# kkoutini/PaSST

Hardware: AMD Instinct MI355X
Metric: clips/s (10s@32k) fwd+bwd passt_s (higher is better)
Workload: dtype bf16; 1 GPU; passt_s_swa_p16_128_ap476 train step (mel front end + mixup + fwd + BCE + bwd + adamw), 768/12/12, 474 tokens (s_patchout_t=40,f=4), random-init weights; global_batch=64, per_gpu_batch=64, parallelism=dp1, gemm_launch=persistent, 256 workgroups, input=waveform (B,1,320000) f32 resident in HBM

## Files before the change

### include/passt_amd.h

```cpp
#ifndef PASST_AMD_H
#define PASST_AMD_H

#include <stdint.h>

#ifdef __cplusplus
extern "C" {
#endif

#define PA_ABI_VERSION 6

enum { PA_F32 = 0, PA_BF16 = 1 };

enum {
    PA_OK = 0,
    PA_EINVAL = -1,
    PA_EUNSUPPORTED = -2,
    PA_ELAUNCH = -3,
    PA_ECOMM = -4
};

int pa_abi_version(void);
const char* pa_error_string(int code);
const char* pa_last_hip_error(void);

// ... 83 lines not shown
    PA_EPI_RESID = 2,
    PA_EPI_DGELU = 3,
    PA_EPI_PARTIAL = 4
};
typedef struct {
    int32_t dtype;
    int32_t epilogue;
    int32_t M, N, K;
    int32_t lda, ldb;
    const void* A;
    const void* B;
    const float* bias;
    const float* resid;
    int32_t ldr;
    int32_t row_mod, out_batch_rows, out_row_off;
    const void* aux;
    int32_t ldaux;
    float* out_f32;
    int32_t ldo32;
    void* out_lp;
    int32_t ldolp;
    void* out_lp2;
    int32_t ldolp2;
    int32_t split_k;
    int32_t tune;
    float* colsum_out;
    float* colsum_ws;
    int32_t colsum_accumulate;
    int32_t reserved;
    int32_t colscale_n;
    float colscale;
} pa_gemm_args;
#define PA_GEMM_BLOCKED_PRE 0x100
#define PA_GEMM_NO_PERSIST 0x400
#define PA_GEMM_EPILOGUE_V3 0x1000
#define PA_GEMM_COLSUM_DEFER 0x2000
int pa_gemm_blocked_pre_ok(int M, int N, int K);
int64_t pa_gemm_blocked_pre_elems(int M, int N);
int64_t pa_gemm_colsum_ws_floats(int M, int N);
int pa_gemm_nt(const pa_gemm_args* a, void* stream);
int pa_gemm_nt_splitk_plan(int M, int N, int K, int epilogue, int dtype);
int64_t pa_gemm_nt_splitk_ws_floats(int M, int N, int K, int epilogue, int dtype);
int pa_gemm_nt_splitk(const pa_gemm_args* a, float* ws, int64_t ws_floats, void* stream);
int pa_gemm_nt_rowscale(const pa_gemm_args* a, const float* rowscale, void* stream);
int pa_gemm_nt_splitk_rowscale(const pa_gemm_args* a, const float* rowscale, float* ws, int64_t ws_floats, void* stream);
int pa_gemm_tn(const pa_gemm_args* a, void* stream);
#define PA_TN_BATCH_MAX 4
#ifndef PA_TN_STEP_ROWS
#define PA_TN_STEP_ROWS 48
#endif
int pa_gemm_tn_step_rows(void);
int pa_gemm_tn_batched(const pa_gemm_args* a, int n, void* stream);
int pa_gemm_tn_batched_plan(const pa_gemm_args* a, int n, int n_long, int long_steps, void* stream);
int pa_gather_rows(const void* in, const int32_t* idx, int n_idx, int64_t row_bytes, void* out, void* stream);
int pa_scatter_rows(const void* in, const int32_t* idx, int n_idx, int64_t row_bytes, void* out, void* stream);
int pa_tail_inject(const float* rows, const int32_t* idx, int n_idx, const float* add0, const float* add1, float* dx,
                   void* dx_lp, int dtype, int M, int D, void* stream);
int pa_zero2d(void* ptr, int64_t pitch_bytes, int64_t width_bytes, int64_t rows, void* stream);
int pa_reduce_partials(const float* partial, int splits, int64_t n, float* out, int accumulate,
                       void* stream);
#define PA_REDUCE_BATCH_MAX 12
#define PA_REDUCE_SLABS 0
#define PA_REDUCE_ROWS 1
typedef struct pa_reduce_desc {
    const float* partial;
    float* out;
    int64_t n;
    int32_t splits;
    int32_t accumulate;
    int64_t pitch;
    int32_t mode;
    int32_t reserved;
} pa_reduce_desc;
int pa_reduce_partials_batched(const pa_reduce_desc* d, int n, void* stream);
int pa_gemm_last_colsum_rows(void);
int pa_rowsum(const void* in, int dtype, int R, int C, int ld, float* out, int accumulate,
              void* stream);
int64_t pa_colsum_ws_floats(int R, int C);
int pa_colsum(const void* in, int dtype, int R, int C, int ld, float* out, int accumulate, float* ws,
              void* stream);
int pa_colsum_f32(const float* in, int R, int C, int ld, float* out, int accumulate, void* stream);

#define PA_ATTN_Q_PRESCALED 1
#define PA_ATTN_BWD_TWO_PASS 2
#define PA_ATTN_BWD_SINGLE_PASS 4
#define PA_ATTN_BWD_SINGLE_PASS_W16 8
int pa_attention_fwd(const void* qkv, int ldqkv, void* o, int ldo, float* lse, int B, int H, int N, int nq,
                     float scale, int dtype, int flags, void* stream);
int pa_attention_fwd_varlen(const void* qkv, int ldqkv, void* o, int ldo, float* lse, const int32_t* cu_tok, int B, int H,
                            int max_N, int nq, float scale, int dtype, int flags, void* stream);
int pa_attention_probs(const void* qkv, int ldqkv, const float* lse, float* out, const int32_t* cu_tok, const int64_t* out_off,
                       int B, int H, int N , int nq, int head_mean, float scale, int dtype, int flags,
                       void* stream);
#define PA_ATTN_PGRAD_GRAD 0
#define PA_ATTN_PGRAD_CAM 1
int pa_attention_probs_grad(const void* qkv, int ldqkv, const float* lse, const void* d_o, int ldo, int do_compact, float* out,
                            const int32_t* cu_tok, const int64_t* out_off, int B, int H, int N , int nq,
                            int head_mean, int mode, float scale, int dtype, int flags, void* stream);
#define PA_ATTN_ROLLOUT_ATTN 0
#define PA_ATTN_ROLLOUT_CAM 1
#define PA_ATTN_ROLLOUT_MAX_ROWS 4
int64_t pa_attention_rollout_ws_floats(int64_t total_tok, int B, int N , int nq, int nr, int slices);
int pa_attention_rollout(const void* qkv, int ldqkv, const float* lse, const void* d_o, int ldo, int do_compact, const float* r_in,
                         float* r_out, float* ws, const int32_t* cu_tok, int64_t total_tok, int B, int H,
                         int N , int nq, int nr, int mode, int slices, float a, float b_, float g_scale,
                         float scale, int dtype, int flags, void* stream);
// ... 118 lines not shown
```

### passt_amd/_lib.py

```python
import ctypes as C
import os

_HERE = os.path.dirname(os.path.abspath(__file__))
LIB_PATH = os.path.join(_HERE, "libpasst_amd.so")
LIB_PATH = os.environ.get("PASST_AMD_LIB", LIB_PATH)

PA_F32, PA_BF16 = 0, 1
EPI_STORE, EPI_GELU, EPI_RESID, EPI_DGELU, EPI_PARTIAL = 0, 1, 2, 3, 4

vp, i32, i64, f32 = C.c_void_p, C.c_int32, C.c_int64, C.c_float


class MelParams(C.Structure):
    _fields_ = [("n_fft", i32), ("hop", i32), ("n_mels", i32), ("n_frames", i32),
                ("preemph", f32), ("mel_low", f32), ("inv_mel_delta", f32), ("log_eps", f32),
                ("out_add", f32), ("out_scale", f32),
                ("fmask_start", i32), ("fmask_end", i32), ("tmask_start", i32), ("tmask_end", i32)]


class MelClipParams(C.Structure):
    _fields_ = [("mel_low", f32), ("inv_mel_delta", f32),
                ("fmask_start", i32), ("fmask_end", i32), ("tmask_start", i32), ("tmask_end", i32)]


# ... 9 lines not shown

class ReduceDesc(C.Structure):
    _fields_ = [("partial", vp), ("out", vp), ("n", i64), ("splits", i32), ("accumulate", i32), ("pitch", i64), ("mode", i32),
                ("reserved", i32)]


class StageDesc(C.Structure):
    _fields_ = [("src", vp), ("dst", vp), ("dst_t", vp), ("rows", i32), ("cols", i32), ("tile_begin", i32), ("reserved", i32)]


class AdamwStageDesc(C.Structure):
    _fields_ = [("offset", i64), ("dst", vp), ("dst_t", vp), ("rows", i32), ("cols", i32), ("tile_begin", i32), ("reserved", i32)]


SIGNATURES = {
    "pa_abi_version": (i32, []),
    "pa_error_string": (C.c_char_p, [i32]),
    "pa_last_hip_error": (C.c_char_p, []),
    "pa_mel_num_frames": (i32, [i32, i32]),
    "pa_mel_frontend_fwd": (i32, [vp, i32, i32, vp, vp, vp, vp, C.POINTER(MelParams), vp]),
    "pa_mel_frontend_fwd_varlen": (i32, [vp, i32, i32, vp, vp, vp, vp, vp, i32, f32, C.POINTER(MelParams), vp]),
    "pa_mel_frontend_bwd": (i32, [vp, i32, i32, vp, vp, vp, vp, vp, vp, i64, C.POINTER(MelParams), vp]),
    "pa_mel_frontend_bwd_varlen": (i32, [vp, i32, i32, vp, vp, vp, vp, vp, i32, vp, vp, i64, C.POINTER(MelParams), vp]),
    "pa_mel_frontend_fwd_varlen_aug": (i32, [vp, i32, i32, vp, vp, vp, vp, vp, i32, f32, C.POINTER(MelParams), vp, vp]),
    "pa_mel_frontend_bwd_varlen_aug": (i32, [vp, i32, i32, vp, vp, vp, vp, vp, i32, vp, vp, i64, C.POINTER(MelParams), vp, vp]),
    "pa_convert_f32": (i32, [vp, vp, i64, i32, vp]),
    "pa_convert_f32_rowscale": (i32, [vp, vp, vp, i32, i32, i32, vp]),
    "pa_convert_to_f32": (i32, [vp, i32, vp, i64, vp]),
    "pa_transpose": (i32, [vp, i32, i32, i32, i32, vp, i32, i32, vp]),
    "pa_stage_weights": (i32, [vp, i32, i32, i32, vp]),
    "pa_layernorm_fwd": (i32, [vp, vp, vp, vp, i32, vp, vp, i32, i32, f32, vp]),
    "pa_layernorm_bwd_ws_floats": (i64, [i32, i32]),
    "pa_layernorm_bwd": (i32, [vp, i32, vp, vp, vp, vp, vp, vp, vp, vp, vp, vp, i32, vp, i32, i32, vp]),
    "pa_layernorm_bwd_rows": (i32, [i32]),
    "pa_layernorm_bwd_partial": (i32, [vp, i32, vp, vp, vp, vp, vp, vp, vp, vp, i32, i32, vp]),
    "pa_layernorm_bwd2": (i32, [vp, i32, vp, vp, vp, vp, vp, vp, vp, vp, vp, vp, vp, i32, vp, i32, i32, vp]),
    "pa_layernorm_bwd2_partial": (i32, [vp, i32, vp, vp, vp, vp, vp, vp, vp, vp, vp, i32, i32, vp]),
    "pa_layernorm_bwd_rowscale": (i32, [vp, i32, vp, vp, vp, vp, vp, vp, vp, vp, vp, vp, vp, vp, i32, vp, i32, i32, vp]),
    "pa_layernorm_bwd_partial_rowscale": (i32, [vp, i32, vp, vp, vp, vp, vp, vp, vp, vp, vp, vp, i32, i32, vp]),
    "pa_tail_inject": (i32, [vp, vp, i32, vp, vp, vp, vp, i32, i32, i32, vp]),
    "pa_gemm_last_colsum_rows": (i32, []),
    "pa_gemm_colsum_ws_floats": (i64, [i32, i32]),
    "pa_gemm_blocked_pre_ok": (i32, [i32, i32, i32]),
    "pa_gemm_blocked_pre_elems": (i64, [i32, i32]),
    "pa_gemm_nt": (i32, [C.POINTER(GemmArgs), vp]),
    "pa_gemm_nt_splitk_plan": (i32, [i32, i32, i32, i32, i32]),
    "pa_gemm_nt_splitk_ws_floats": (i64, [i32, i32, i32, i32, i32]),
    "pa_gemm_nt_splitk": (i32, [C.POINTER(GemmArgs), vp, i64, vp]),
    "pa_gemm_nt_rowscale": (i32, [C.POINTER(GemmArgs), vp, vp]),
    "pa_gemm_nt_splitk_rowscale": (i32, [C.POINTER(GemmArgs), vp, vp, i64, vp]),
    "pa_gemm_tn": (i32, [C.POINTER(GemmArgs), vp]),
    "pa_gemm_tn_batched": (i32, [C.POINTER(GemmArgs), i32, vp]),
    "pa_gemm_tn_batched_plan": (i32, [C.POINTER(GemmArgs), i32, i32, i32, vp]),
    "pa_gemm_tn_step_rows": (i32, []),
    "pa_reduce_partials_batched": (i32, [C.POINTER(ReduceDesc), i32, vp]),
    "pa_colsum_ws_floats": (i64, [i32, i32]),
    "pa_colsum": (i32, [vp, i32, i32, i32, i32, vp, i32, vp, vp]),
    "pa_reduce_partials": (i32, [vp, i32, i64, vp, i32, vp]),
    "pa_rowsum": (i32, [vp, i32, i32, i32, i32, vp, i32, vp]),
    "pa_colsum_f32": (i32, [vp, i32, i32, i32, vp, i32, vp]),
    "pa_attention_fwd": (i32, [vp, i32, vp, i32, vp, i32, i32, i32, i32, f32, i32, i32, vp]),
    "pa_attention_fwd_varlen": (i32, [vp, i32, vp, i32, vp, vp, i32, i32, i32, i32, f32, i32, i32, vp]),
    "pa_attention_probs": (i32, [vp, i32, vp, vp, vp, vp, i32, i32, i32, i32, i32, f32, i32, i32, vp]),
    "pa_attention_probs_grad": (i32, [vp, i32, vp, vp, i32, i32, vp, vp, vp, i32, i32, i32, i32, i32, i32, f32, i32, i32, vp]),
    "pa_attention_rollout_ws_floats": (i64, [i64, i32, i32, i32, i32, i32]),
    "pa_attention_rollout": (i32, [vp, i32, vp, vp, i32, i32, vp, vp, vp, vp, i64, i32, i32, i32, i32, i32, i32, i32, f32, f32, f32, f32,
                                   i32, i32, vp]),
    "pa_attention_bwd_ws_floats": (i64, [i32, i32, i32]),
    "pa_attention_bwd": (i32, [vp, i32, vp, vp, i32, vp, vp, vp, i32, i32, i32, i32, i32, f32, i32, i32, vp]),
    "pa_attention_bwd_varlen_ws_floats": (i64, [i64, i32, i32, i32]),
    "pa_attention_bwd_varlen": (i32, [vp, i32, vp, vp, i32, vp, vp, vp, i32, vp, i32, i32, i32, i32, f32, i32, i32, vp]),
    "pa_gather_rows": (i32, [vp, vp, i32, i64, vp, vp]),
    "pa_scatter_rows": (i32, [vp, vp, i32, i64, vp, vp]),
    "pa_zero2d": (i32, [vp, i64, i64, i64, vp]),
    "pa_patch_gather": (i32, [vp, i32, i32, i32, vp, vp, i32, i32, i32, i32, vp, i32, vp]),
    "pa_patch_pos_table": (i32, [vp, vp, i32, vp, i32, vp, vp, i32, i32, i32, vp, vp, vp, vp, vp, i32, i32, vp]),
    "pa_patch_gather_varlen": (i32, [vp, i32, i32, i32, vp, vp, vp, i32, i32, i32, i32, vp, i32, vp]),
    "pa_patch_pos_table_varlen": (i32, [vp, vp, i32, vp, i32, vp, vp, i32, i32, vp, vp, vp, vp, vp]),
    "pa_patch_input_bwd_varlen": (i32, [vp, i32, vp, i32, i32, i32, i32, i32, i32, vp, vp]),
    "pa_patch_bwd_varlen": (i32, [vp, i32, i32, vp, i32, i32, i32, vp, vp, vp, vp, vp, vp, i32, vp]),
    "pa_patch_input_bwd_rows": (i32, [vp, i32, i32, vp, i32, i32, i32, i32, i32, i32, i32, vp, vp]),
    "pa_patch_bwd_rows": (i32, [vp, i32, i32, vp, vp, vp, i32, i32, i32, i32, vp, vp, vp, vp, vp, vp, i32, vp]),
    "pa_patch_bwd": (i32, [vp, i32, i32, i32, vp, vp, i32, i32, i32, i32, vp, vp, vp, vp, vp, vp, vp, i32, vp, i32, vp]),
    "pa_patch_input_bwd_ws_ints": (i64, [i32, i32, i32, i32, i32]),
    "pa_patch_input_bwd": (i32, [vp, i32, i32, i32, vp, vp, i32, i32, i32, i32, i32, vp, vp, vp]),
    "pa_head_pre_fwd": (i32, [vp, i32, i32, i32, vp, vp, f32, vp, vp, f32, vp, vp, vp, vp]),
    "pa_linear_f32_fwd": (i32, [vp, vp, vp, vp, i32, i32, i32, vp]),
    "pa_linear_f32_bwd": (i32, [vp, vp, vp, vp, vp, vp, i32, i32, i32, i32, vp]),
    "pa_head_pre_bwd": (i32, [vp, vp, vp, vp, i32, i32, i32, vp, vp, vp, vp, vp, vp]),
    "pa_bce_fwd_bwd": (i32, [vp, vp, i32, i32, f32, vp, vp, vp, vp]),
    "pa_ce_mixup_fwd_bwd": (i32, [vp, vp, vp, vp, i32, i32, f32, vp, vp, vp, vp]),
    "pa_mixup": (i32, [vp, vp, vp, vp, i32, i64, vp]),
    "pa_adamw": (i32, [vp, vp, vp, vp, i64, f32, f32, f32, f32, f32, i32, vp]),
    "pa_adamw_dev": (i32, [vp, vp, vp, vp, i64, vp, vp]),
    "pa_adamw_stage": (i32, [vp, vp, vp, vp, vp, i32, i32, i32, f32, f32, f32, f32, f32, i32, vp, vp]),
    "pa_adamw_stage_groups": (i32, [vp, vp, vp, vp, vp, vp, i32, i32, i32, f32, f32, f32, f32, f32, i32, vp, vp]),
    "pa_adamw_groups": (i32, [vp, vp, vp, vp, vp, vp, i32, i32, f32, f32, f32, f32, f32, i32, vp, vp]),
    "pa_grad_norm_partials": (i64, [i64]),
    "pa_grad_accum_sumsq": (i32, [vp, vp, i32, i64, vp, vp]),
    "pa_clip_coef": (i32, [vp, i32, f32, vp, vp]),
    "pa_adamw_clip": (i32, [vp, vp, vp, vp, i64, f32, f32, f32, f32, f32, i32, vp, vp, vp]),
    "pa_adamw_stage_clip": (i32, [vp, vp, vp, vp, vp, vp, i32, i32, i32, f32, f32, f32, f32, f32, i32, vp, vp, vp]),
    "pa_adamw_hyper": (None, [f32, f32, f32, f32, f32, i32, C.POINTER(f32)]),
    "pa_sgd": (i32, [vp, vp, i64, f32, vp]),
    "pa_swa_update": (i32, [vp, vp, i64, i32, vp]),
    "pa_wave_augment": (i32, [vp, i32, i64, vp, vp, vp, vp, vp, vp, vp, i64, vp]),
    "pa_ir_conv_plan": (i32, [i32, C.POINTER(i32), C.POINTER(i32)]),
    "pa_ir_bank_floats": (i64, [i32, i32]),
    "pa_ir_bank_prepare": (i32, [vp, i32, i32, vp, vp, vp]),
    "pa_wave_ir_convolve": (i32, [vp, i32, i64, vp, vp, vp, vp, i32, i32, vp, i64, i64, vp, vp]),
    "pa_eval_append": (i32, [vp, vp, vp, i32, i32, i64, i64, i32, vp, vp, vp]),
    "pa_eval_ws_bytes": (i64, [i32, i64]),
    "pa_eval_rank": (i32, [vp, vp, i32, i64, i64, vp, vp, vp, vp, vp, vp, vp]),
    "pa_comm_unique_id": (i32, [vp]),
    "pa_comm_init": (i32, [vp, i32, i32, C.POINTER(vp)]),
    "pa_allreduce_bucket": (i32, [vp, vp, i64, i32, vp]),
    "pa_comm_destroy": (i32, [vp]),
    "pa_comm_info": (i32, [vp, C.POINTER(i32), C.POINTER(i32), C.POINTER(i32), C.POINTER(i32)]),
    "pa_comm_last_error": (C.c_char_p, []),
}
GEMM_BLOCKED_PRE = 0x100
GEMM_NO_PERSIST = 0x400
GEMM_COLSUM_DEFER = 0x2000
REDUCE_SLABS, REDUCE_ROWS = 0, 1
GEMM_EPILOGUE_V3 = 0x1000
COMM_ID_BYTES = 128
EVAL_SIGMOID, EVAL_RAW = 0, 1
EVAL_EXCLUDED, EVAL_NEG, EVAL_POS, EVAL_NAN = 0, 1, 2, 3

_lib = None


class PasstAmdError(RuntimeError):
    pass


def load():
    global _lib
    if _lib is not None:
        return _lib
    if not os.path.isfile(LIB_PATH):
        raise PasstAmdError(
            f"{LIB_PATH} not found: the HIP extension is not built.  Run "
            "`make -C passt_amd/csrc` (needs hipcc, --offload-arch=gfx950).  passt_amd has no CPU fallback.")
    lib = C.CDLL(LIB_PATH)
    for name, (res, args) in SIGNATURES.items():
        fn = getattr(lib, name)
        fn.restype, fn.argtypes = res, args
    if lib.pa_abi_version() != 6:
        raise PasstAmdError("libpasst_amd.so ABI version mismatch; rebuild")
    _lib = lib
    return lib


def compile_opaque(fn):
    import functools

    import torch
    try:
        ef = torch._C._dynamo.eval_frame
        set_eval_frame = ef.set_eval_frame
        skip = ef._FrameExecStrategy(ef._FrameAction.SKIP, ef._FrameAction.DEFAULT)
    except AttributeError:
        return torch.compiler.disable(fn)

    @functools.wraps(fn)
    def opaque_forward(*args, **kwargs):
        prior = set_eval_frame(None)
        try:
            return fn(*args, **kwargs)
        finally:
            set_eval_frame(prior)

    ef.set_code_exec_strategy(opaque_forward.__code__, skip)
    opaque_forward._torchdynamo_disable = True
# ... 15 lines not shown
```

### passt_amd/csrc/gemm.hip

```cpp
#include <algorithm>
#include <cstring>
#include <type_traits>

#include "pa_mma.h"

namespace pa {

static constexpr int NT_GROUP_M = 4;
static constexpr int BM = 128, BN = 128, KB = 128;
static constexpr int TILE_BYTES = BM * KB;
static constexpr int GEMM_LDS = 2 * 2 * TILE_BYTES;

#ifdef PA_PROBE
__device__ unsigned long long* g_probe_buf = nullptr;
static constexpr int PROBE_SLOTS = 512;
#define PA_PROBE_STAMP(cond, idx)                                                                             \
    do {                                                                                                      \
        if ((cond) && (wave & 3) == 0 && lane == 0 && (idx) < PROBE_SLOTS)                                    \
            ((unsigned long long*)(smem + G::LDS))[(wave >> 2) * PROBE_SLOTS + (idx)] = __builtin_amdgcn_s_memtime(); \
    } while (0)
#define PA_PROBE_FLAG(a, bit) (((a).reserved >> (bit)) & 1)
#define PA_PROBE_STAMP_TN(cond, idx)                                                                          \
    do {                                                                                                      \
        if ((cond) && (wave & 3) == 0 && lane == 0 && (idx) < PROBE_SLOTS)                                    \
            ((unsigned long long*)(smem + TN_LDS))[(wave >> 2) * PROBE_SLOTS + (idx)] = __builtin_amdgcn_s_memtime(); \
    } while (0)
#else
#define PA_PROBE_STAMP(cond, idx) do {} while (0)
#define PA_PROBE_STAMP_TN(cond, idx) do {} while (0)
#define PA_PROBE_FLAG(a, bit) 0
#endif


static constexpr int SLAB_BYTES = 32 * 68 * 4;

static int finish_gemm_colsum(const pa_gemm_args& a, int rows, hipStream_t st);

template <int EPI, int TM> __host__ __device__ constexpr int aux_depth() {
    return EPI == PA_EPI_DGELU ? TM : (EPI == PA_EPI_RESID ? (TM <= 3 ? TM : 2) : 0);
}

template <int EPI>
__device__ __forceinline__ void load_bias8(const pa_gemm_args& a, int n0, int wc, int lane, float (&bias8)[8]) {
    const int ncol = n0 + wc * 64 + (lane & 7) * 8;
#pragma unroll
    for (int e = 0; e < 8; ++e) bias8[e] = 0.f;
    if constexpr (EPI != PA_EPI_PARTIAL && EPI != PA_EPI_DGELU) {
        if (a.bias && ncol < a.N) {
            const f32x4 lo = *(const f32x4*)(a.bias + ncol), hi = *(const f32x4*)(a.bias + ncol + 4);
#pragma unroll
            for (int e = 0; e < 4; ++e) { bias8[e] = lo[e]; bias8[4 + e] = hi[e]; }
        }
    }
}

// ... 1645 lines not shown
    gemm_tn_stagger_item(a, tiles_n, xcd_swizzle(blockIdx.x, nwg), blockIdx.y, steps_per_split);
}

struct TnBatch {
    pa_gemm_args a[PA_TN_BATCH_MAX];
    int32_t first[PA_TN_BATCH_MAX + 1];
    int32_t tiles_n[PA_TN_BATCH_MAX], nwg[PA_TN_BATCH_MAX], per[PA_TN_BATCH_MAX];
    int32_t tfirst[PA_TN_BATCH_MAX + 1];
    int32_t n, order;
};
__global__ __launch_bounds__(512) void gemm_tn_stagger_batched_kernel(const TnBatch b) {
    int p = 0, t, split;
    if (b.order == 1) {
        const int logical = xcd_swizzle(blockIdx.x, b.first[b.n]);
        const int tiles_all = b.tfirst[b.n];
        split = logical / tiles_all;
        t = logical - split * tiles_all;
        while (p + 1 < b.n && t >= b.tfirst[p + 1]) ++p;
        t -= b.tfirst[p];
    } else {
        while (p + 1 < b.n && (int)blockIdx.x >= b.first[p + 1]) ++p;
        const int item = blockIdx.x - b.first[p];
        split = item / b.nwg[p];
        t = xcd_swizzle(item - split * b.nwg[p], b.nwg[p]);
    }
    gemm_tn_stagger_item(b.a[p], b.tiles_n[p], t, split, b.per[p]);
}

struct TnPlan {
    pa_gemm_args a[PA_TN_BATCH_MAX];
    int32_t tiles_n[PA_TN_BATCH_MAX];
    int32_t tfirst[PA_TN_BATCH_MAX + 1];
    int32_t n, n_long, long_steps, steps;
};
__global__ __launch_bounds__(512) void gemm_tn_stagger_plan_kernel(const TnPlan b) {
    const int tiles_all = b.tfirst[b.n], nlong = tiles_all * b.n_long;
    int g, t;
    if ((int)blockIdx.x < nlong) {
        const int logical = xcd_swizzle(blockIdx.x, nlong);
        g = logical / tiles_all;
        t = logical - g * tiles_all;
    } else {
        g = b.n_long;
        t = xcd_swizzle(blockIdx.x - nlong, tiles_all);
    }
    int p = 0;
    while (p + 1 < b.n && t >= b.tfirst[p + 1]) ++p;
    t -= b.tfirst[p];
    const pa_gemm_args& a = b.a[p];
    const int st_begin = g * b.long_steps;
    const int nsteps = g < b.n_long ? b.long_steps : b.steps - st_begin;
    gemm_tn_stagger_range(a, b.tiles_n[p], t, st_begin, nsteps, a.out_f32 + (int64_t)g * a.M * a.ldo32, a.ldo32,
                          a.colsum_ws ? a.colsum_ws + (int64_t)g * a.M : nullptr);
}

static int launch_gemm_tn_stagger(const pa_gemm_args& a, hipStream_t st) {
#ifdef PA_PROBE
    constexpr int LDS = TN_LDS + 2 * PROBE_SLOTS * 8;
#else
    constexpr int LDS = TN_LDS;
#endif
    const int tiles_m = (int)cdiv(a.M, 256), tiles_n = (int)cdiv(a.N, 256);
    const int nwg = tiles_m * tiles_n;
    const int steps = (int)cdiv(a.K, TN_ROWS);
    const int per = (int)cdiv(steps, a.split_k);
    static signed char lds_attr[64] = {0};
    (void)lds_attr_on_this_device((const void*)gemm_tn_stagger_kernel, LDS, lds_attr);
    hipLaunchKernelGGL(gemm_tn_stagger_kernel, dim3(nwg, a.split_k), dim3(512), LDS, st, a, tiles_n, nwg, per);
    return check_launch();
}

template <typename T>
static int launch_gemm_tn(const pa_gemm_args& a, hipStream_t st) {
    const int tiles_m = (int)cdiv(a.M, BM), tiles_n = (int)cdiv(a.N, BN);
    const int nwg = tiles_m * tiles_n;
    const int steps = (int)cdiv(a.K, TNGeom<T>::MROWS);
    const int per = (int)cdiv(steps, a.split_k);
    static signed char lds_attr[64] = {0};
    (void)lds_attr_on_this_device((const void*)gemm_tn_kernel<T>, GEMM_LDS, lds_attr);
    hipLaunchKernelGGL((gemm_tn_kernel<T>), dim3(nwg, a.split_k), dim3(256), GEMM_LDS, st, a, tiles_n, nwg, per);
    return check_launch();
}

template <typename T>
__global__ __launch_bounds__(256) void colsum_stage1_kernel(const T* __restrict__ in, int R, int C, int ld,
                                                            float* __restrict__ part, int rows_per_block) {
    __shared__ float red[32][65];
    const int tx = threadIdx.x & 7, ty = threadIdx.x >> 3;
    const int c0 = blockIdx.x * 64 + tx * 8;
    const int r_begin = blockIdx.y * rows_per_block, r_end = min(R, r_begin + rows_per_block);
    float s[8];
#pragma unroll
    for (int e = 0; e < 8; ++e) s[e] = 0.f;
    for (int r = r_begin + ty; r < r_end; r += 32) {
        float v[8];
        if (c0 < C) {
            load8<T>(in + (int64_t)r * ld + c0, v);
#pragma unroll
            for (int e = 0; e < 8; ++e) s[e] += v[e];
        }
    }
#pragma unroll
    for (int e = 0; e < 8; ++e) red[ty][tx * 8 + e] = s[e];
    __syncthreads();
    if (threadIdx.x < 64) {
        float t = 0.f;
// ... 489 lines not shown
        tiles += pb->nwg[p];
        same_split = same_split && x.split_k == a[0].split_k;
    }
    pb->first[n] = total;
    pb->tfirst[n] = tiles;
    pb->n = n;
    pb->order = (a[0].tune != 2 && same_split) ? 1 : 0;
#ifdef PA_PROBE
    constexpr int LDS = TN_LDS + 2 * PROBE_SLOTS * 8;
#else
    constexpr int LDS = TN_LDS;
#endif
    static signed char lds_attr[64] = {0};
    (void)lds_attr_on_this_device((const void*)gemm_tn_stagger_batched_kernel, LDS, lds_attr);
    hipLaunchKernelGGL(gemm_tn_stagger_batched_kernel, dim3(total), dim3(512), LDS, (hipStream_t)stream, batch);
    return check_launch();
}

extern "C" int pa_gemm_tn_batched_plan(const pa_gemm_args* a, int n, int n_long, int long_steps, void* stream) {
    if (!a || n < 1 || n > PA_TN_BATCH_MAX || n_long < 1 || long_steps < 1) return PA_EINVAL;
    TnPlan plan;
    TnPlan* pb = &plan;
    int64_t tiles = 0;
    for (int p = 0; p < n; ++p) {
        const pa_gemm_args& x = a[p];
        if (!x.A || !x.B || !x.out_f32 || x.M <= 0 || x.N <= 0 || x.K <= 0 || x.split_k != n_long + 1) return PA_EINVAL;
        if (x.dtype != PA_BF16 || x.epilogue != PA_EPI_PARTIAL) return PA_EUNSUPPORTED;
        if ((x.lda * 2) % 16 || (x.ldb * 2) % 16 || x.ldo32 % 4 || x.M < 8 || x.N < 8 || x.N % 8 || x.M % 8) return PA_EUNSUPPORTED;
        if (x.K != a[0].K) return PA_EUNSUPPORTED;
        pb->a[p] = x;
        pb->tiles_n[p] = (int)cdiv(x.N, 256);
        pb->tfirst[p] = (int)tiles;
        tiles += cdiv(x.M, 256) * pb->tiles_n[p];
    }
    const int steps = (int)cdiv(a[0].K, TN_ROWS);
    if ((int64_t)n_long * long_steps >= steps) return PA_EINVAL;
    if (tiles * (n_long + 1) > INT32_MAX) return PA_EUNSUPPORTED;
    pb->tfirst[n] = (int)tiles;
    pb->n = n;
    pb->n_long = n_long;
    pb->long_steps = long_steps;
    pb->steps = steps;
#ifdef PA_PROBE
    constexpr int LDS = TN_LDS + 2 * PROBE_SLOTS * 8;
#else
    constexpr int LDS = TN_LDS;
#endif
    static signed char lds_attr[64] = {0};
    (void)lds_attr_on_this_device((const void*)gemm_tn_stagger_plan_kernel, LDS, lds_attr);
    hipLaunchKernelGGL(gemm_tn_stagger_plan_kernel, dim3((unsigned)(tiles * (n_long + 1))), dim3(512), LDS, (hipStream_t)stream, plan);
    return check_launch();
}

namespace pa {
struct ReduceBatch {
    pa_reduce_desc d[PA_REDUCE_BATCH_MAX];
    int32_t n;
};
__global__ __launch_bounds__(256) void reduce_partials_batched_kernel(const ReduceBatch b) {
    const pa_reduce_desc& d = b.d[blockIdx.y];
    if (d.mode == PA_REDUCE_ROWS) {
        __shared__ float red[16][17];
        const int cx = threadIdx.x & 15, ry = threadIdx.x >> 4;
        for (int64_t c0 = (int64_t)blockIdx.x * 16; c0 < d.n; c0 += (int64_t)gridDim.x * 16) {
            const int64_t k = c0 + cx;
            float s = 0.f, s1 = 0.f, s2 = 0.f, s3 = 0.f;
            if (k < d.n) {
                int r = ry;
                for (; r + 48 < d.splits; r += 64) {
                    s += d.partial[(int64_t)r * d.pitch + k];
                    s1 += d.partial[(int64_t)(r + 16) * d.pitch + k];
                    s2 += d.partial[(int64_t)(r + 32) * d.pitch + k];
                    s3 += d.partial[(int64_t)(r + 48) * d.pitch + k];
                }
                for (; r < d.splits; r += 16) s += d.partial[(int64_t)r * d.pitch + k];
            }
            red[ry][cx] = (s + s1) + (s2 + s3);
            __syncthreads();
            if (ry == 0 && k < d.n) {
                float t = 0.f;
#pragma unroll
                for (int y = 0; y < 16; ++y) t += red[y][cx];
                d.out[k] = (d.accumulate ? d.out[k] : 0.f) + t;
            }
            __syncthreads();
        }
        return;
    }
    const int64_t n = d.n, n4 = (n % 4 == 0 && (((uintptr_t)d.partial | (uintptr_t)d.out) & 15) == 0) ? n / 4 : 0;
    const int64_t stride = (int64_t)gridDim.x * blockDim.x, t0 = (int64_t)blockIdx.x * blockDim.x + threadIdx.x;
    for (int64_t i = t0; i < n4; i += stride) {
        f32x4 s = d.accumulate ? ((const f32x4*)d.out)[i] : f32x4{0.f, 0.f, 0.f, 0.f};
        for (int z = 0; z < d.splits; ++z) {
            if constexpr (CP_NT_SLAB_LOADS) s += __builtin_nontemporal_load((const f32x4*)(d.partial + (int64_t)z * n + i * 4));
            else s += *(const f32x4*)(d.partial + (int64_t)z * n + i * 4);
        }
        ((f32x4*)d.out)[i] = s;
    }
    for (int64_t i = n4 * 4 + t0; i < n; i += stride) {
        float s = d.accumulate ? d.out[i] : 0.f;
        for (int z = 0; z < d.splits; ++z) s += d.partial[(int64_t)z * n + i];
        d.out[i] = s;
    }
}
}

// ... 84 lines not shown
```

### passt_amd/ops.py

```python
import collections
import ctypes as C
import functools
import threading
import os

import numpy as np
import torch

from . import _lib
from ._lib import (GEMM_BLOCKED_PRE, EPI_DGELU, EPI_GELU, EPI_PARTIAL, EPI_RESID, EPI_STORE, PA_BF16, PA_F32,
                   GemmArgs, MelParams, check)

TORCH_DTYPE = {PA_F32: torch.float32, PA_BF16: torch.bfloat16}
PA_DTYPE = {torch.float32: PA_F32, torch.bfloat16: PA_BF16}


class _CallState(threading.local):
    dev = None
    gemm_flags = 0


_call = _CallState()


# ... 586 lines not shown
    need = S * N * K
    if partial_ws is None or partial_ws.numel() < need:
        partial_ws = torch.empty(need, device=dY_t.device, dtype=torch.float32)
    part = partial_ws[:need].view(S, N, K)
    gemm_nt(dY_t, X_t, dtype, EPI_PARTIAL, out_f32=part, split_k=S)
    check(_lib.load().pa_reduce_partials(_p(part), S, N * K, _p(out_f32), int(accumulate), _stream()),
          "pa_reduce_partials")
    return partial_ws


def tn_step_rows():
    return _lib.load().pa_gemm_tn_step_rows()



def pick_split_k_slots(tiles, steps, slots=256):
    best, best_score = 1, -1.0
    for S in range(1, max(1, min(64, steps // 8)) + 1):
        blocks = tiles * S
        eff = blocks / (((blocks + slots - 1) // slots) * slots)
        score = eff - 0.003 * S
        if score > best_score:
            best, best_score = S, score
    return best


_SPLITS_CACHE = {}
_FORCE_SLICES = int(os.environ.get("PASST_AMD_WGRAD_SLICES", "0"))


def pick_batched_splits(probs, slots=256):
    key = (tuple(probs), slots)
    hit = _SPLITS_CACHE.get(key)
    if hit is None:
        hit = _SPLITS_CACHE[key] = _pick_batched_splits(list(probs), slots)
        if _FORCE_SLICES:
            hit = _SPLITS_CACHE[key] = [max(1, min(_FORCE_SLICES, st)) for _, st in probs]
    return hit


def _pick_batched_splits(probs, slots=256):
    best, best_cost = None, None
    for L in range(max(p[1] for p in probs), 3, -1):
        S = [max(1, min(64, -(-st // L))) for _, st in probs]
        items = sum(t * s_ for (t, _), s_ in zip(probs, S))
        per = max(-(-st // s_) for (_, st), s_ in zip(probs, S))
        cost = -(-items // slots) * (per + 4) * 1.2 + items * 0.05
        if best_cost is None or cost < best_cost - 1e-9:
            best, best_cost = S, cost
    return best if best is not None else [1] * len(probs)


_PLAN_CACHE = {}
WGRAD_PLAN_DEFAULT = "long_short"
_SHORT_ITEM_COST = 1.25
_PLAN_MIN_GAIN = 0.04
_FORCE_UNIFORM = os.environ.get("PASST_AMD_WGRAD_PLAN", WGRAD_PLAN_DEFAULT) == "uniform" or _FORCE_SLICES > 0


def pick_batched_plan(probs, slots=256):
    if _FORCE_UNIFORM:
        return 0, 0, pick_batched_splits(probs, slots)
    key = (tuple(probs), slots)
    hit = _PLAN_CACHE.get(key)
    if hit is None:
        hit = _PLAN_CACHE[key] = _pick_batched_plan(list(probs), slots)
    return hit


def _uniform_cost(probs, S, slots=256):
    items = sum(t * s_ for (t, _), s_ in zip(probs, S))
    per = max(-(-st // s_) for (_, st), s_ in zip(probs, S))
    return -(-items // slots) * (per + 4) * 1.2 + items * 0.05


def _long_short_cost(tiles, steps, a, L, slots=256):
    import heapq
    free = [0.0] * slots
    end = 0.0
    for steps_item, count, k in ((L, a * tiles, 1.0), (steps - a * L, tiles, _SHORT_ITEM_COST)):
        dur = (steps_item + 4) * 1.2 * k
        for _ in range(count):
            t = free[0] + dur
            heapq.heapreplace(free, t)
            end = max(end, t)
    return end + tiles * (a + 1) * 0.05


def _pick_batched_plan(probs, slots=256):
    S = _pick_batched_splits(probs, slots)
    steps = probs[0][1]
    tiles = sum(t for t, _ in probs)
    if any(st != steps for _, st in probs) or sum(t * s_ for (t, _), s_ in zip(probs, S)) <= slots:
        return 0, 0, S
    best, best_cost = (0, 0, S), _uniform_cost(probs, S, slots)
    for a in (1, 2):
        for L in range((steps - 1) // a, -(-steps // (a + 1)) - 1, -1):
            cost = _long_short_cost(tiles, steps, a, L, slots)
            if cost < best_cost - 1e-9:
                best, best_cost = (a, L, [a + 1] * len(probs)), cost
    return best if best_cost < (1.0 - _PLAN_MIN_GAIN) * _uniform_cost(probs, S, slots) else (0, 0, S)


def wgrad_batched_ws_floats(splits, shapes):
    return sum(S * N * (K + (1 if has_db else 0)) for S, (N, K, has_db) in zip(splits, shapes))


def wgrad_tn(dY, X, out_f32, dtype, accumulate=False, partial_ws=None, db=None):
    Mtok, N = dY.shape
    K = X.shape[1]
    if dtype == PA_BF16 and GEMM_TUNE != 1:
        tiles = ((N + 255) // 256) * ((K + 255) // 256)
        S = pick_split_k_slots(tiles, (Mtok + tn_step_rows() - 1) // tn_step_rows())
    else:
        tiles = ((N + 127) // 128) * ((K + 127) // 128)
        mrows = 64 if dtype == PA_BF16 else 32
        S = pick_split_k(tiles, (Mtok + mrows - 1) // mrows)
    assert db is None or wgrad_tn_fuses_bias(dtype)
    need = S * N * K + (S * N if db is not None else 0)
    if partial_ws is None or partial_ws.numel() < need:
        partial_ws = torch.empty(need, device=dY.device, dtype=torch.float32)
    part = partial_ws[:S * N * K].view(S, N, K)
    a = GemmArgs()
    a.dtype, a.epilogue = dtype, EPI_PARTIAL
    a.M, a.N, a.K = N, K, Mtok
    a.lda, a.ldb = dY.stride(0), X.stride(0)
    a.A, a.B = _p(dY, dtype, True), _p(X, dtype, True)
    a.out_f32, a.ldo32 = _p(part), K
    a.split_k = S
    a.tune = GEMM_TUNE
    bpart = partial_ws[S * N * K:need] if db is not None else None
    a.colsum_ws = _p(bpart)
    lib = _lib.load()
    ev0 = ev1 = None
    if GEMM_PROFILE is not None:
        ev0, ev1 = torch.cuda.Event(enable_timing=True), torch.cuda.Event(enable_timing=True)
        ev0.record()
    check(lib.pa_gemm_tn(C.byref(a), _stream()), "pa_gemm_tn")
    check(lib.pa_reduce_partials(_p(part), S, N * K, _p(out_f32), int(accumulate), _stream()), "pa_reduce_partials")
    if db is not None:
        check(lib.pa_reduce_partials(_p(bpart), S, N, _p(db, torch.float32), int(accumulate), _stream()), "pa_reduce_partials")
    if ev0 is not None:
        ev1.record()
        GEMM_PROFILE.setdefault("wgrad_tn", []).append((ev0, ev1, 2.0 * N * K * Mtok))
    return partial_ws


def wgrad_tn_fuses_bias(dtype):
    return dtype == PA_BF16 and GEMM_TUNE != 1


def wgrad_tn_batched(problems, dtype, partial_ws=None, row_jobs=None, plan=None):
    from ._lib import ReduceDesc
    assert dtype == PA_BF16 and 1 <= len(problems) <= 4
    problems = [tuple(p) + (None,) * (5 - len(p)) for p in problems]
    metas = []
    for dY, X, out, acc, db in problems:
        Mtok, N = dY.shape
        metas.append((Mtok, N, X.shape[1]))
    shapes = [(((N + 255) // 256) * ((K + 255) // 256), (Mtok + tn_step_rows() - 1) // tn_step_rows()) for Mtok, N, K in metas]
    if plan is None:
        n_long, long_steps, splits = pick_batched_plan(shapes)
    elif plan[0] == 0:
        n_long, long_steps, splits = 0, 0, pick_batched_splits(shapes)
    else:
        n_long, long_steps = plan
        splits = [n_long + 1] * len(problems)
    need = wgrad_batched_ws_floats(splits, [(m[1], m[2], p[4] is not None) for m, p in zip(metas, problems)])
    if partial_ws is None or partial_ws.numel() < need:
        partial_ws = torch.empty(need, device=problems[0][0].device, dtype=torch.float32)
    row_jobs = row_jobs or []
    nred = len(problems) + sum(1 for p in problems if p[4] is not None) + len(row_jobs)
    args = (GemmArgs * len(problems))()
    red = (ReduceDesc * nred)()
    off, flops, k = 0, 0.0, len(problems)
    for a, r, (dY, X, out, acc, db), (Mtok, N, K), S in zip(args, red, problems, metas, splits):
        part = partial_ws[off:off + S * N * K]
        off += S * N * K
        a.dtype, a.epilogue = dtype, EPI_PARTIAL
        a.M, a.N, a.K = N, K, Mtok
        a.lda, a.ldb = dY.stride(0), X.stride(0)
        a.A, a.B = _p(dY, dtype, True), _p(X, dtype, True)
        a.out_f32, a.ldo32 = _p(part), K
        a.split_k, a.tune = S, TN_BATCH_ORDER
        r.partial, r.out, r.n, r.splits, r.accumulate = _p(part), _p(out, torch.float32), N * K, S, int(acc)
        if db is not None:
            bpart = partial_ws[off:off + S * N]
            off += S * N
            a.colsum_ws = _p(bpart)
            rb = red[k]
            k += 1
            rb.partial, rb.out, rb.n, rb.splits, rb.accumulate = _p(bpart), _p(db, torch.float32), N, S, int(acc)
        flops += 2.0 * N * K * Mtok
    for part_rows, rows, pitch, n, out in row_jobs:
        rb = red[k]
        k += 1
        rb.partial, rb.out, rb.n, rb.splits, rb.accumulate = _p(part_rows, torch.float32, True), _p(out, torch.float32), n, rows, 0
        rb.pitch, rb.mode = pitch, _lib.REDUCE_ROWS
    lib = _lib.load()
    ev0 = ev1 = None
    if GEMM_PROFILE is not None:
        ev0, ev1 = torch.cuda.Event(enable_timing=True), torch.cuda.Event(enable_timing=True)
        ev0.record()
    if n_long:
        check(lib.pa_gemm_tn_batched_plan(args, len(problems), n_long, long_steps, _stream()), "pa_gemm_tn_batched_plan")
    else:
        check(lib.pa_gemm_tn_batched(args, len(problems), _stream()), "pa_gemm_tn_batched")
    for lo in range(0, nred, REDUCE_BATCH_MAX):
        n = min(REDUCE_BATCH_MAX, nred - lo)
        check(lib.pa_reduce_partials_batched(C.cast(C.byref(red, lo * C.sizeof(ReduceDesc)), C.POINTER(ReduceDesc)), n, _stream()),
              "pa_reduce_partials_batched")
    if ev0 is not None:
        ev1.record()
        GEMM_PROFILE.setdefault("wgrad_tn", []).append((ev0, ev1, flops))
    return partial_ws


REDUCE_BATCH_MAX = 12


def colsum(x, out_f32, accumulate=False):
    R, Cc = x.shape
    lib = _lib.load()
    ws = torch.empty(lib.pa_colsum_ws_floats(R, Cc), device=x.device, dtype=torch.float32)
    check(lib.pa_colsum(_p(x, None, True), PA_DTYPE[x.dtype], R, Cc, x.stride(0), _p(out_f32, torch.float32), int(accumulate), _p(ws),
                        _stream()), "pa_colsum")


def rowsum(x, out_f32, ncols=None, accumulate=False):
    R, Cc = x.shape
    check(_lib.load().pa_rowsum(_p(x, None, True), PA_DTYPE[x.dtype], R, Cc if ncols is None else ncols, x.stride(0),
                                _p(out_f32), int(accumulate), _stream()), "pa_rowsum")


def colsum_f32(x, out_f32, accumulate=False):
    R, Cc = x.shape
    check(_lib.load().pa_colsum_f32(_p(x, torch.float32, True), R, Cc, x.stride(0), _p(out_f32, torch.float32), int(accumulate), _stream()),
          "pa_colsum_f32")


ATTN_Q_PRESCALED = 1
ATTN_BWD_TWO_PASS = 2
ATTN_BWD_SINGLE_PASS = 4
ATTN_BWD_SINGLE_PASS_W16 = 8
_ATTN_BWD_FORCE = {"two_pass": ATTN_BWD_TWO_PASS, "single_pass": ATTN_BWD_SINGLE_PASS,
                   "single_pass_w16": ATTN_BWD_SINGLE_PASS_W16}.get(os.environ.get("PASST_AMD_ATTN_BWD", ""), 0)
LOG2E = 1.4426950408889634


def attention_fwd(qkv, B, H, N, scale, nq=None, flags=0):
    dtype = PA_DTYPE[qkv.dtype]
    nq = N if nq is None else nq
    D = H * 64
    o = torch.empty((B * nq, D), device=qkv.device, dtype=qkv.dtype)
    lse = torch.empty((B * H * nq,), device=qkv.device, dtype=torch.float32)
    _timed("attn_fwd", 4.0 * nq * N * 64 * B * H,
           lambda: check(_lib.load().pa_attention_fwd(_p(qkv, None, True), qkv.stride(0), _p(o), o.stride(0), _p(lse), B, H, N, nq,
# ... 589 lines not shown
```

Measured before the change: 2996 clips/s.

## Add dealt per-workgroup work lists for batched wgrad TN GEMM scheduling

Adds a host-built, cached table that assigns each of the 256 persistent workgroups an explicit list of (problem, tile, step range) items. Long split-K chunks are dealt round-robin and the short remainders go to the least-loaded slot, with the goal of balancing the batched weight-gradient GEMM better than the uniform long/short plan. It becomes the default wgrad plan whenever its modeled cost beats the uniform plan. The cost is a device-side table read per item, a one-time hipMalloc plus memcpy per shape, and a fallback when the stream is being graph-captured.

```diff
diff --git a/include/passt_amd.h b/include/passt_amd.h
--- a/include/passt_amd.h
+++ b/include/passt_amd.h
@@ -159,6 +159,11 @@
 int pa_gemm_tn_step_rows(void);
 int pa_gemm_tn_batched(const pa_gemm_args* a, int n, void* stream);
 int pa_gemm_tn_batched_plan(const pa_gemm_args* a, int n, int n_long, int long_steps, void* stream);
+#define PA_TN_DEALT_MAX_LIST 8
+#define PA_TN_DEALT_ENTRY_INTS 5
+#define PA_TN_DEALT_STRIDE (1 + PA_TN_DEALT_MAX_LIST * PA_TN_DEALT_ENTRY_INTS)
+int pa_gemm_tn_batched_dealt(const pa_gemm_args* a, int n, int n_long, int long_steps, int slots, void* stream);
+int pa_tn_dealt_table(const int32_t* tiles, int n, int steps, int n_long, int long_steps, int slots, int32_t* out);
 int pa_gather_rows(const void* in, const int32_t* idx, int n_idx, int64_t row_bytes, void* out, void* stream);
 int pa_scatter_rows(const void* in, const int32_t* idx, int n_idx, int64_t row_bytes, void* out, void* stream);
 int pa_tail_inject(const float* rows, const int32_t* idx, int n_idx, const float* add0, const float* add1, float* dx,
diff --git a/passt_amd/_lib.py b/passt_amd/_lib.py
--- a/passt_amd/_lib.py
+++ b/passt_amd/_lib.py
@@ -85,6 +85,8 @@
     "pa_gemm_tn": (i32, [C.POINTER(GemmArgs), vp]),
     "pa_gemm_tn_batched": (i32, [C.POINTER(GemmArgs), i32, vp]),
     "pa_gemm_tn_batched_plan": (i32, [C.POINTER(GemmArgs), i32, i32, i32, vp]),
+    "pa_gemm_tn_batched_dealt": (i32, [C.POINTER(GemmArgs), i32, i32, i32, i32, vp]),
+    "pa_tn_dealt_table": (i32, [C.POINTER(C.c_int32), i32, i32, i32, i32, i32, C.POINTER(C.c_int32)]),
     "pa_gemm_tn_step_rows": (i32, []),
     "pa_reduce_partials_batched": (i32, [C.POINTER(ReduceDesc), i32, vp]),
     "pa_colsum_ws_floats": (i64, [i32, i32]),
@@ -154,6 +156,8 @@
 }
 GEMM_BLOCKED_PRE = 0x100
 GEMM_NO_PERSIST = 0x400
+TN_DEALT_MAX_LIST, TN_DEALT_ENTRY_INTS = 8, 5
+TN_DEALT_STRIDE = 1 + TN_DEALT_MAX_LIST * TN_DEALT_ENTRY_INTS
 GEMM_COLSUM_DEFER = 0x2000
 REDUCE_SLABS, REDUCE_ROWS = 0, 1
 GEMM_EPILOGUE_V3 = 0x1000
diff --git a/passt_amd/csrc/gemm.hip b/passt_amd/csrc/gemm.hip
--- a/passt_amd/csrc/gemm.hip
+++ b/passt_amd/csrc/gemm.hip
@@ -1,6 +1,9 @@
 #include <algorithm>
 #include <cstring>
+#include <map>
+#include <mutex>
 #include <type_traits>
+#include <vector>
 
 #include "pa_mma.h"
 
@@ -1752,6 +1755,25 @@
     const int nsteps = g < b.n_long ? b.long_steps : b.steps - st_begin;
     gemm_tn_stagger_range(a, b.tiles_n[p], t, st_begin, nsteps, a.out_f32 + (int64_t)g * a.M * a.ldo32, a.ldo32,
                           a.colsum_ws ? a.colsum_ws + (int64_t)g * a.M : nullptr);
+}
+
+struct TnDealt {
+    pa_gemm_args a[PA_TN_BATCH_MAX];
+    int32_t tiles_n[PA_TN_BATCH_MAX];
+    const int32_t* table;
+};
+__global__ __launch_bounds__(512) void gemm_tn_stagger_dealt_kernel(const TnDealt b) {
+    const int32_t* row = b.table + (int64_t)blockIdx.x * PA_TN_DEALT_STRIDE;
+    const int count = __builtin_amdgcn_readfirstlane(row[0]);
+    for (int i = 0; i < count; ++i) {
+        const int32_t* e = row + 1 + i * PA_TN_DEALT_ENTRY_INTS;
+        const int p = __builtin_amdgcn_readfirstlane(e[0]), t = __builtin_amdgcn_readfirstlane(e[1]);
+        const int st_begin = __builtin_amdgcn_readfirstlane(e[2]), nsteps = __builtin_amdgcn_readfirstlane(e[3]);
+        const int g = __builtin_amdgcn_readfirstlane(e[4]);
+        const pa_gemm_args& a = b.a[p];
+        gemm_tn_stagger_range(a, b.tiles_n[p], t, st_begin, nsteps, a.out_f32 + (int64_t)g * a.M * a.ldo32, a.ldo32,
+                              a.colsum_ws ? a.colsum_ws + (int64_t)g * a.M : nullptr);
+    }
 }
 
 static int launch_gemm_tn_stagger(const pa_gemm_args& a, hipStream_t st) {
@@ -2347,6 +2369,120 @@
     return check_launch();
 }
 
+extern "C" int pa_tn_dealt_table(const int32_t* tiles, int n, int steps, int n_long, int long_steps, int slots, int32_t* out) {
+    if (!tiles || !out || n < 1 || n > PA_TN_BATCH_MAX || n_long < 1 || long_steps < 1 || slots < 1 || steps < 1) return PA_EINVAL;
+    if ((int64_t)n_long * long_steps >= steps) return PA_EINVAL;
+    int64_t tiles_all = 0;
+    int tfirst[PA_TN_BATCH_MAX + 1];
+    for (int p = 0; p < n; ++p) {
+        if (tiles[p] < 1) return PA_EINVAL;
+        tfirst[p] = (int)tiles_all;
+        tiles_all += tiles[p];
+    }
+    if (tiles_all * (n_long + 1) > (int64_t)slots * PA_TN_DEALT_MAX_LIST) return PA_EUNSUPPORTED;
+    tfirst[n] = (int)tiles_all;
+    const int nx = std::min(8, slots), short_steps = steps - n_long * long_steps;
+    const int64_t nlong = tiles_all * n_long;
+    for (int s = 0; s < slots; ++s) out[(int64_t)s * PA_TN_DEALT_STRIDE] = 0;
+    std::vector<int64_t> load((size_t)slots, 0);
+    int longest = 0;
+    auto push = [&](int s, int64_t t_all, int g, int nsteps) {
+        int32_t* row = out + (int64_t)s * PA_TN_DEALT_STRIDE;
+        if (row[0] >= PA_TN_DEALT_MAX_LIST) return false;
+        int p = 0;
+        while (p + 1 < n && t_all >= tfirst[p + 1]) ++p;
+        int32_t* e = row + 1 + row[0] * PA_TN_DEALT_ENTRY_INTS;
+        e[0] = p, e[1] = (int)(t_all - tfirst[p]), e[2] = g * long_steps, e[3] = nsteps, e[4] = g;
+        longest = std::max(longest, ++row[0]);
+        load[(size_t)s] += nsteps + 4;
+        return true;
+    };
+    auto run = [&](int64_t total, int x, int64_t& first, int64_t& len) {
+        const int64_t q = total / nx, r = total % nx;
+        first = x < r ? x * (q + 1) : r * (q + 1) + (x - r) * q;
+        len = q + (x < r ? 1 : 0);
+    };
+    for (int x = 0; x < nx; ++x) {
+        const int cx = (slots - x + nx - 1) / nx;
+        int64_t first, len;
+        run(nlong, x, first, len);
+        for (int64_t j = 0; j < len; ++j) {
+            const int64_t logical = first + j;
+            if (!push(x + (int)(j % cx) * nx, logical % tiles_all, (int)(logical / tiles_all), long_steps)) return PA_EUNSUPPORTED;
+        }
+        run(tiles_all, x, first, len);
+        for (int64_t j = 0; j < len; ++j) {
+            int best = 0;
+            for (int c = 1; c < cx; ++c)
+                if (load[(size_t)(x + c * nx)] < load[(size_t)(x + best * nx)]) best = c;
+            if (!push(x + best * nx, first + j, n_long, short_steps)) return PA_EUNSUPPORTED;
+        }
+    }
+    return longest;
+}
+
+namespace pa {
+static const int32_t* tn_dealt_table_on_device(const int32_t* tiles, int n, int steps, int n_long, int long_steps, int slots, hipStream_t st,
+                                               int* rc) {
+    static std::mutex mu;
+    static std::map<std::vector<int>, const int32_t*> cache;
+    int dev = 0;
+    hipError_t e = hipGetDevice(&dev);
+    if (e != hipSuccess) { *rc = set_hip_error(e); return nullptr; }
+    std::vector<int> key{dev, steps, n_long, long_steps, slots};
+    key.insert(key.end(), tiles, tiles + n);
+    std::lock_guard<std::mutex> lock(mu);
+    auto hit = cache.find(key);
+    if (hit != cache.end()) return hit->second;
+    std::vector<int32_t> host((size_t)slots * PA_TN_DEALT_STRIDE, 0);
+    const int longest = pa_tn_dealt_table(tiles, n, steps, n_long, long_steps, slots, host.data());
+    if (longest < 0) { *rc = longest; return nullptr; }
+    hipStreamCaptureStatus cap = hipStreamCaptureStatusNone;
+    if (hipStreamIsCapturing(st, &cap) != hipSuccess || cap != hipStreamCaptureStatusNone) { *rc = PA_OK; return nullptr; }
+    void* d = nullptr;
+    e = hipMalloc(&d, host.size() * sizeof(int32_t));
+    if (e == hipSuccess) {
+        e = hipMemcpy(d, host.data(), host.size() * sizeof(int32_t), hipMemcpyHostToDevice);
+        if (e != hipSuccess) (void)hipFree(d);
+    }
+    if (e != hipSuccess) { *rc = set_hip_error(e); return nullptr; }
+    return cache[key] = (const int32_t*)d;
+}
+}
+
+extern "C" int pa_gemm_tn_batched_dealt(const pa_gemm_args* a, int n, int n_long, int long_steps, int slots, void* stream) {
+    if (!a || n < 1 || n > PA_TN_BATCH_MAX || n_long < 1 || long_steps < 1 || slots < 1) return PA_EINVAL;
+    TnDealt plan;
+    TnDealt* pb = &plan;
+    int32_t tiles[PA_TN_BATCH_MAX];
+    for (int p = 0; p < n; ++p) {
+        const pa_gemm_args& x = a[p];
+        if (!x.A || !x.B || !x.out_f32 || x.M <= 0 || x.N <= 0 || x.K <= 0 || x.split_k != n_long + 1) return PA_EINVAL;
+        if (x.dtype != PA_BF16 || x.epilogue != PA_EPI_PARTIAL) return PA_EUNSUPPORTED;
+        if ((x.lda * 2) % 16 || (x.ldb * 2) % 16 || x.ldo32 % 4 || x.M < 8 || x.N < 8 || x.N % 8 || x.M % 8) return PA_EUNSUPPORTED;
+        if (x.K != a[0].K) return PA_EUNSUPPORTED;
+        pb->a[p] = x;
+        pb->tiles_n[p] = (int)cdiv(x.N, 256);
+        const int64_t t = cdiv(x.M, 256) * pb->tiles_n[p];
+        if (t > INT32_MAX / 4) return PA_EUNSUPPORTED;
+        tiles[p] = (int32_t)t;
+    }
+    const int steps = (int)cdiv(a[0].K, TN_ROWS);
+    if ((int64_t)n_long * long_steps >= steps) return PA_EINVAL;
+    int rc = PA_OK;
+    pb->table = tn_dealt_table_on_device(tiles, n, steps, n_long, long_steps, slots, (hipStream_t)stream, &rc);
+    if (!pb->table) return rc != PA_OK ? rc : pa_gemm_tn_batched_plan(a, n, n_long, long_steps, stream);
+#ifdef PA_PROBE
+    constexpr int LDS = TN_LDS + 2 * PROBE_SLOTS * 8;
+#else
+    constexpr int LDS = TN_LDS;
+#endif
+    static signed char lds_attr[64] = {0};
+    (void)lds_attr_on_this_device((const void*)gemm_tn_stagger_dealt_kernel, LDS, lds_attr);
+    hipLaunchKernelGGL(gemm_tn_stagger_dealt_kernel, dim3((unsigned)slots), dim3(512), LDS, (hipStream_t)stream, plan);
+    return check_launch();
+}
+
 namespace pa {
 struct ReduceBatch {
     pa_reduce_desc d[PA_REDUCE_BATCH_MAX];
diff --git a/passt_amd/ops.py b/passt_amd/ops.py
--- a/passt_amd/ops.py
+++ b/passt_amd/ops.py
@@ -662,7 +662,7 @@
 
 
 _PLAN_CACHE = {}
-WGRAD_PLAN_DEFAULT = "long_short"
+WGRAD_PLAN_DEFAULT = "dealt"
 _SHORT_ITEM_COST = 1.25
 _PLAN_MIN_GAIN = 0.04
 _FORCE_UNIFORM = os.environ.get("PASST_AMD_WGRAD_PLAN", WGRAD_PLAN_DEFAULT) == "uniform" or _FORCE_SLICES > 0
@@ -710,6 +710,51 @@
             if cost < best_cost - 1e-9:
                 best, best_cost = (a, L, [a + 1] * len(probs)), cost
     return best if best_cost < (1.0 - _PLAN_MIN_GAIN) * _uniform_cost(probs, S, slots) else (0, 0, S)
+
+
+_DEALT_ENABLED = os.environ.get("PASST_AMD_WGRAD_PLAN", WGRAD_PLAN_DEFAULT) == "dealt" and not _FORCE_UNIFORM
+_DEALT_CACHE = {}
+
+
+def dealt_lists(tiles, steps, n_long, long_steps, slots=256):
+    lib = _lib.load()
+    stride, ints = _lib.TN_DEALT_STRIDE, _lib.TN_DEALT_ENTRY_INTS
+    out = (C.c_int32 * (slots * stride))()
+    rc = lib.pa_tn_dealt_table((C.c_int32 * len(tiles))(*tiles), len(tiles), steps, n_long, long_steps, slots, out)
+    if rc < 0:
+        check(rc, "pa_tn_dealt_table")
+    return [[tuple(out[s * stride + 1 + i * ints:s * stride + 1 + (i + 1) * ints]) for i in range(out[s * stride])] for s in range(slots)]
+
+
+def _dealt_cost(probs, a, L, slots=256):
+    lists = dealt_lists([t for t, _ in probs], probs[0][1], a, L, slots)
+    return max(sum(e[3] + 4 for e in lst) for lst in lists) * 1.2 + sum(t for t, _ in probs) * (a + 1) * 0.05
+
+
+def _pick_dealt_plan(probs, slots=256):
+    S = _pick_batched_splits(probs, slots)
+    steps = probs[0][1]
+    if any(st != steps for _, st in probs) or sum(t * s_ for (t, _), s_ in zip(probs, S)) <= slots:
+        return None
+    best, best_cost = None, (1.0 - _PLAN_MIN_GAIN) * _uniform_cost(probs, S, slots)
+    for a in (1, 2):
+        if sum(t for t, _ in probs) * (a + 1) > slots * _lib.TN_DEALT_MAX_LIST:
+            continue
+        for L in range((steps - 1) // a, -(-steps // (a + 1)) - 1, -1):
+            cost = _dealt_cost(probs, a, L, slots)
+            if cost < best_cost - 1e-9:
+                best, best_cost = (a, L, [a + 1] * len(probs)), cost
+    return best
+
+
+def pick_wgrad_launch(probs, slots=256):
+    if _DEALT_ENABLED:
+        key = (tuple(probs), slots)
+        if key not in _DEALT_CACHE:
+            _DEALT_CACHE[key] = _pick_dealt_plan(list(probs), slots)
+        if _DEALT_CACHE[key] is not None:
+            return (True,) + _DEALT_CACHE[key]
+    return (False,) + tuple(pick_batched_plan(probs, slots))
 
 
 def wgrad_batched_ws_floats(splits, shapes):
@@ -760,7 +805,7 @@
     return dtype == PA_BF16 and GEMM_TUNE != 1
 
 
-def wgrad_tn_batched(problems, dtype, partial_ws=None, row_jobs=None, plan=None):
+def wgrad_tn_batched(problems, dtype, partial_ws=None, row_jobs=None, plan=None, dealt=None, slots=256):
     from ._lib import ReduceDesc
     assert dtype == PA_BF16 and 1 <= len(problems) <= 4
     problems = [tuple(p) + (None,) * (5 - len(p)) for p in problems]
@@ -769,8 +814,10 @@
         Mtok, N = dY.shape
         metas.append((Mtok, N, X.shape[1]))
     shapes = [(((N + 255) // 256) * ((K + 255) // 256), (Mtok + tn_step_rows() - 1) // tn_step_rows()) for Mtok, N, K in metas]
-    if plan is None:
-        n_long, long_steps, splits = pick_batched_plan(shapes)
+    if plan is None and not (_call.gemm_flags & _lib.GEMM_NO_PERSIST):
+        dealt, n_long, long_steps, splits = pick_wgrad_launch(shapes, slots)
+    elif plan is None:
+        dealt, (n_long, long_steps, splits) = False, pick_batched_plan(shapes)
     elif plan[0] == 0:
         n_long, long_steps, splits = 0, 0, pick_batched_splits(shapes)
     else:
@@ -812,7 +859,9 @@
     if GEMM_PROFILE is not None:
         ev0, ev1 = torch.cuda.Event(enable_timing=True), torch.cuda.Event(enable_timing=True)
         ev0.record()
-    if n_long:
+    if n_long and dealt:
+        check(lib.pa_gemm_tn_batched_dealt(args, len(problems), n_long, long_steps, slots, _stream()), "pa_gemm_tn_batched_dealt")
+    elif n_long:
         check(lib.pa_gemm_tn_batched_plan(args, len(problems), n_long, long_steps, _stream()), "pa_gemm_tn_batched_plan")
     else:
         check(lib.pa_gemm_tn_batched(args, len(problems), _stream()), "pa_gemm_tn_batched")
```

Result: no change. 3006 clips/s (median of 6 runs) (+0.3%).
